# HarmoniaLeo/FRLW-EvD

Hardware: AMD Instinct MI355X
Metric: TAF encode throughput (Mevents/s) (higher is better)
Workload: dtype f32

## Files before the change

frlw-evd_amd/csrc/taf_split.h:

```cpp
#pragma once
#include "taf_column.h"
#include "taf_partition.h"
#include <type_traits>

namespace {
struct TileP {
    int H, W, twl, thl, tiles_x, T, K, n_windows, wb, flip;
    uint32_t win;
    const uint32_t *rec;
    uint32_t *rec2;
    const uint32_t *base;
    uint32_t *sub;
    uint32_t *sub_end;
    const uint32_t *seg0;
    uint32_t *segcnt;
    int pairs;
    int direct;
    int seg_grid;
    uint32_t tile_max;
    const float *tlut;
    const uint32_t *leaky_thr;
    FastHeader *hdr;
    double rcp;
    float *state;
    float *view_f32;
    uint8_t *out_u8;
    uint32_t *wst, *wst_flag;
};

__device__ __forceinline__ int pair_of_segment(const uint32_t *seg0, int pairs, uint32_t seg)
{
    int lo = 0, hi = pairs;
    while (hi - lo > 1) {
        const int mid = (lo + hi) >> 1;
        if (seg0[mid] <= seg) lo = mid; else hi = mid;
    }
    return lo;
}

__device__ __forceinline__ void count_subtiles(const uint32_t *rec, uint32_t beg, uint32_t end, uint32_t (*wtot)[kFW])
{
    const int tid = threadIdx.x, wv = tid >> 6;
    for (uint32_t c0 = beg; c0 < end; c0 += 8 * kFT) {
        uint32_t v[8];
#pragma unroll
        for (int u = 0; u < 8; ++u) {
            const uint32_t i = c0 + (uint32_t)(u * kFT + tid);
            v[u] = rec[i < end ? i : end - 1u];
        }
#pragma unroll
        for (int u = 0; u < 8; ++u)
            if (c0 + (uint32_t)(u * kFT + tid) < end) atomicAdd(&wtot[wv][(v[u] & (kCells - 1)) >> 8], 1u);
    }
}

__device__ __forceinline__ void split_count_segment(const TileP &q, uint32_t seg, uint32_t (*wtot)[kFW])
{
    const int tid = threadIdx.x, wv = tid >> 6;
    if (seg >= q.seg0[q.pairs]) return;
    const int g = pair_of_segment(q.seg0, q.pairs, seg);
    const uint32_t beg = q.base[g] + (seg - q.seg0[g]) * (uint32_t)kSplitSeg;
    const uint32_t end = q.base[g + 1] - beg < (uint32_t)kSplitSeg ? q.base[g + 1] : beg + kSplitSeg;
    if (tid < kFW * kFW) (&wtot[0][0])[tid] = 0u;
    __syncthreads();
    count_subtiles(q.rec, beg, end, wtot);
    __syncthreads();
    if (tid < kFW) {
        uint32_t t = 0;
#pragma unroll
        for (int w = 0; w < kFW; ++w) t += wtot[w][tid];
        q.segcnt[(long long)seg * kFW + tid] = t;
    }
}

constexpr int kWholeChunks = FRLW_WHOLE_SEGS;
constexpr int kWholeBatches = kWholeChunks * kSplitSeg / kWave;
constexpr int kWholeRow = kWholeBatches + 1;

template <bool CM>
__global__ __launch_bounds__(kFT) __attribute__((amdgpu_waves_per_eu(8, 8))) void kf_split_whole(TileP q, CmP cm, SeqTab S)
{
    constexpr int RPT = kSplitSeg / kFT;
    constexpr int kColWords = 2 * kColMax + 1 + kSplitWhole / 32 + 1;
    constexpr int kPoolTail = CM && kColWords > kSplitSeg ? kColWords - kSplitSeg : 0;
    __shared__ __attribute__((aligned(16))) uint32_t pool[kFW * kWholeRow + kSplitSeg + kPoolTail];
    uint32_t *scnt = pool, *stage = pool + kFW * kWholeRow;
    __shared__ uint32_t wtot[kFW][kFW];
    __shared__ uint32_t vtot[kFW];
    __shared__ uint32_t vbeg[kFW][kFW];
    __shared__ uint32_t cE[kFW][kFW], cD[kFW][kFW];
    __shared__ uint32_t s_start, s_first;
    __shared__ int s_unsorted;
    __shared__ int s_fw[kWholeChunks][kFW], s_lw[kWholeChunks][kFW];
    __shared__ uint32_t s_wst[CM ? kFW * (FRLW_MAX_WINDOWS + 1) : 1];
    const int tid = threadIdx.x, lane = tid & 63, wv = tid >> 6;
    const int32_t status0 = q.hdr->status;
    if (!CM && status0 != 0) return;
    const int blk = (int)blockIdx.x;
    if (!CM && blk >= q.pairs) {
        const uint32_t nseg = q.seg0[q.pairs];
        for (uint32_t seg = (uint32_t)(blk - q.pairs); seg < nseg; seg += (uint32_t)q.seg_grid) {
            split_count_segment(q, seg, wtot);
            __syncthreads();
        }
        return;
    }
    const int g = CM ? (int)xcd_owned_index(blockIdx.x, gridDim.x) : blk;
    uint32_t beg, n;
    uint32_t m[kWholeChunks][RPT];
    if (CM) {
        uint32_t *colL = stage, *colD = stage + kColMax + 1;
        uint16_t *idx = (uint16_t *)(stage + 2 * kColMax + 1);
        const int s = g / q.T, C = S.chunk0[s + 1] - S.chunk0[s];
        for (int i = tid; i < kFW * kWholeRow; i += kFT) scnt[i] = 0u;
        n = col_load<kFT>(cm, S, s, g - s * q.T, colL, colD, &wtot[0][0]);
        if (status0 != 0) return;
        if (n == 0u) {
            if (tid < kFW) { q.sub[(long long)g * kFW + tid] = 0u; q.sub_end[(long long)g * kFW + tid] = 0u; }
            if (q.wst && tid == 0) q.wst_flag[g] = 0u;
            return;
        }
        const bool hot = n > q.tile_max;
        if (tid == 0) {
            s_start = atomicAdd(&q.hdr->rec_cursor, n);
            if (hot) s_first = atomicAdd(&q.hdr->seg_cursor, (n + kSplitSeg - 1) / kSplitSeg);
            if (q.wst && hot) q.wst_flag[g] = 0u;
            s_unsorted = 0;
        }
        if (q.wst && !hot) {
            if (tid < kWholeChunks * kFW) { (&s_fw[0][0])[tid] = -1; (&s_lw[0][0])[tid] = -1; }
            for (int i = tid; i < kFW * (q.n_windows + 1); i += kFT) s_wst[i] = 0xffffffffu;
        }
        if (hot) {
            __syncthreads();
            const uint32_t nseg = (n + kSplitSeg - 1) / kSplitSeg, first = s_first;
            if (tid == 0) { cm.hot_start[g] = s_start; cm.hot_seg0[g] = first; }
            for (uint32_t k = tid; k < nseg; k += kFT)
                if (first + k < (uint32_t)cm.max_segs) cm.segdesc[first + k] = (uint32_t)g;
            return;
        }
        col_index<kFT>(colL, C, 0u, n, idx);
        __syncthreads();
        const uint32_t wvs = (uint32_t)__builtin_amdgcn_readfirstlane(wv);
        {
            const __amdgpu_buffer_rsrc_t rsrc = __builtin_amdgcn_make_buffer_rsrc((void *)cm.rec, 0, 0xffffffffu, 0x00020000);
#pragma unroll
            for (int c = 0; c < kWholeChunks; ++c) {
#pragma unroll
                for (int u = 0; u < RPT; ++u) {
                    const uint32_t i = (uint32_t)(c * kSplitSeg + u * kFT + tid), ic = i < n ? i : n - 1u;
                    const uint32_t i0 = (uint32_t)(c * kSplitSeg + u * kFT) + wvs * kWave;
                    uint32_t off = 0u;
                    if (i0 < n) {
                        const uint32_t last = i0 + 63u < n ? i0 + 63u : n - 1u;
                        uint32_t cs = (uint32_t)__builtin_amdgcn_readfirstlane((int)idx[i0 >> 4]);
                        uint32_t lnext = (uint32_t)__builtin_amdgcn_readfirstlane((int)colL[cs + 1]);
                        while (lnext <= i0) { ++cs; lnext = (uint32_t)__builtin_amdgcn_readfirstlane((int)colL[cs + 1]); }
                        if (lnext > last) off = (uint32_t)__builtin_amdgcn_readfirstlane((int)colD[cs]) + ic;
                        else off = col_addr(colL, colD, idx[ic >> 4], ic);
                    }
                    m[c][u] = (uint32_t)__builtin_amdgcn_raw_buffer_load_b32(rsrc, (int)(off << 2), 0, 0);
                }
            }
        }
        beg = (uint32_t)__builtin_amdgcn_readfirstlane((int)s_start);
    } else {
        beg = q.base[g];
        const uint32_t end = q.base[g + 1];
        if (g == q.pairs - 1 && tid == 0) q.sub[(long long)q.pairs * kFW] = end;
        if (end - beg > whole_max_of(q.pairs)) return;
        n = end - beg;
        if (n == 0u) {
            if (tid < kFW) q.sub[(long long)g * kFW + tid] = beg;
            return;
        }
#pragma unroll
        for (int c = 0; c < kWholeChunks; ++c)
#pragma unroll
            for (int u = 0; u < RPT; ++u) {
                const uint32_t i = (uint32_t)(c * kSplitSeg + u * kFT + tid);
                m[c][u] = q.rec[beg + (i < n ? i : n - 1u)];
            }
    }
    if (!CM) {
        for (int i = tid; i < kFW * kWholeRow; i += kFT) scnt[i] = 0u;
        __syncthreads();
    }
    uint32_t rk[kWholeChunks][RPT / 4];
#pragma unroll
    for (int c = 0; c < kWholeChunks; ++c) {
#pragma unroll
        for (int u4 = 0; u4 < RPT / 4; ++u4) rk[c][u4] = 0u;
#pragma unroll
        for (int u = 0; u < RPT; ++u) {
            const uint32_t i0 = (uint32_t)(c * kSplitSeg + u * kFT + wv * kWave);
            if (i0 < n) {
                const bool valid = i0 + (uint32_t)lane < n;
                const uint32_t b = valid ? (m[c][u] & (kCells - 1)) >> 8 : (uint32_t)(lane & 15);
                const uint32_t t = atomicAdd(&scnt[b * kWholeRow + (c * RPT + u) * kFW + wv], valid ? 1u : 0u);
                rk[c][u >> 2] |= t << (8 * (u & 3));
            }
        }
    }
    __syncthreads();
    {
        uint32_t carry = 0;
#pragma unroll
        for (int k = 0; k < kWholeBatches / kWave; ++k) {
            if ((uint32_t)(k * kWave * kWave) < n) {
                const uint32_t v = scnt[wv * kWholeRow + k * kWave + lane];
                const uint32_t inc = wave_incl_scan(v);
                scnt[wv * kWholeRow + k * kWave + lane] = carry + inc - v;
                carry += __shfl(inc, kWave - 1);
            }
        }
        if (lane == 0) vtot[wv] = carry;
    }
    __syncthreads();
    {
        const uint32_t t = vtot[lane & 15];
        uint32_t inc = t;
#pragma unroll
        for (int o2 = 1; o2 < kFW; o2 <<= 1) {
            const uint32_t u = __shfl_up(inc, o2);
            if ((lane & 15) >= o2) inc += u;
        }
        if (lane < kFW) {
            vbeg[wv][lane] = beg + inc - t;
            if (wv == 0) {
                q.sub[(long long)g * kFW + lane] = beg + inc - t;
                if (CM) q.sub_end[(long long)g * kFW + lane] = beg + inc;
            }
        }
        LDS_FENCE();
    }
    const bool wtab = CM && q.wst != nullptr;
#pragma unroll
    for (int c = 0; c < kWholeChunks; ++c) {
        if ((uint32_t)(c * kSplitSeg) >= n) break;
        const uint32_t nch = n - (uint32_t)(c * kSplitSeg) < (uint32_t)kSplitSeg ? n - (uint32_t)(c * kSplitSeg) : (uint32_t)kSplitSeg;
        {
            const int b = lane & 15;
            const uint32_t p0 = scnt[b * kWholeRow + c * (kSplitSeg / kWave)];
            const uint32_t p1 = (uint32_t)((c + 1) * kSplitSeg) < n ? scnt[b * kWholeRow + (c + 1) * (kSplitSeg / kWave)] : vtot[b];
            const uint32_t cnt = p1 - p0;
            uint32_t inc = cnt;
#pragma unroll
            for (int o2 = 1; o2 < kFW; o2 <<= 1) {
                const uint32_t u = __shfl_up(inc, o2);
                if (b >= o2) inc += u;
            }
            if (lane < kFW) {
                cE[wv][lane] = (inc - cnt) - p0;
                cD[wv][lane] = vbeg[wv][lane] + p0 - (inc - cnt);
            }
            LDS_FENCE();
        }
#pragma unroll
        for (int u = 0; u < RPT; ++u) {
            const uint32_t i = (uint32_t)(u * kFT + tid);
            if (i < nch) {
                const uint32_t b = (m[c][u] & (kCells - 1)) >> 8;
                const uint32_t t = (rk[c][u >> 2] >> (8 * (u & 3))) & 255u;
                stage[cE[wv][b] + scnt[b * kWholeRow + (c * RPT + u) * kFW + wv] + t] = m[c][u];
            }
        }
        __syncthreads();
#pragma unroll
        for (int u = 0; u < RPT; ++u) {
            const uint32_t i = (uint32_t)(u * kFT + tid);
            if (i < nch) {
                const uint32_t r = stage[i];
                q.rec2[cD[wv][(r & (kCells - 1)) >> 8] + i] = r;
            }
        }
        if (wtab) {
            const uint32_t dmask = (((1u << q.wb) - 1u) << kCellBits) | (uint32_t)(kCells - 1) >> 8 << 8;
            uint32_t cand = 0u;
#pragma unroll
            for (int u0 = 0; u0 < RPT; u0 += 2) {
                uint32_t r[2], rp[2];
#pragma unroll
                for (int k = 0; k < 2; ++k) {
                    const uint32_t i = (uint32_t)((u0 + k) * kFT + tid);
                    r[k] = stage[i];
                    rp[k] = stage[(i - 1u) & (kSplitSeg - 1)];
                }
#pragma unroll
                for (int k = 0; k < 2; ++k) asm volatile("" : "+v"(r[k]), "+v"(rp[k]));
#pragma unroll
                for (int k = 0; k < 2; ++k) {
                    const uint32_t i = (uint32_t)((u0 + k) * kFT + tid);
                    cand |= (i < nch && (((r[k] ^ rp[k]) & dmask) != 0u || i == 0u || i == nch - 1u) ? 1u : 0u) << (u0 + k);
                }
            }
            while (cand) {
                const int u = __builtin_ctz(cand);
                cand &= cand - 1u;
                const uint32_t i = (uint32_t)(u * kFT + tid);
                const uint32_t r = stage[i], rp = stage[i > 0u ? i - 1u : 0u];
                const int bsub = (int)((r & (kCells - 1)) >> 8), bp = (int)((rp & (kCells - 1)) >> 8);
                const int wc = (int)__builtin_amdgcn_ubfe(r, kCellBits, q.wb), wpn = (int)__builtin_amdgcn_ubfe(rp, kCellBits, q.wb);
                const bool same = i > 0u && bp == bsub;
                if (!same || wc != wpn) atomicMin(&s_wst[bsub * (q.n_windows + 1) + wc], cD[wv][bsub] + i - vbeg[wv][bsub]);
                if (same && wc < wpn) s_unsorted = 1;
                if (!same) { s_fw[c][bsub] = wc; if (i > 0u) s_lw[c][bp] = wpn; }
                if (i == nch - 1u) s_lw[c][bsub] = wc;
            }
        }
        if (wtab && (uint32_t)((c + 1) * kSplitSeg) >= n) LDS_BARRIER();
        else __syncthreads();
    }
    if (wtab) {
        if (tid < kFW) {
            int prev = -1;
            for (int c = 0; c < kWholeChunks; ++c)
                if (s_fw[c][tid] >= 0) { if (s_fw[c][tid] < prev) s_unsorted = 1; prev = s_lw[c][tid]; }
        }
        uint32_t *const wr = q.wst + (long long)g * kFW * (q.n_windows + 1);
        for (int i = tid; i < kFW * (q.n_windows + 1); i += kFT) wr[i] = s_wst[i];
        LDS_BARRIER();
        if (tid == 0) q.wst_flag[g] = s_unsorted ? 2u : 1u;
    }
}

constexpr int kSplitRpt = kSplitSeg / kFT;
struct PlaceLds {
    uint32_t scnt[kSplitRpt][kFW][kFW];
    uint32_t vtot[kFW];
    uint32_t stot[kFW], sdst[kFW];
    uint32_t cE[kFW][kFW], cD[kFW][kFW];
    uint32_t stage[kSplitSeg];
};

struct ColLds {
    uint32_t L[kColMax + 1], D[kColMax];
    uint16_t idx[kSplitSeg / 16];
    uint32_t wsum[kFW + 1];
};

template <bool CM>
__device__ __forceinline__ void split_place_segment(const TileP &q, uint32_t seg, PlaceLds &L, const CmP &cm, const SeqTab &S, ColLds *cl)
{
    constexpr int RPT = kSplitRpt, NE = RPT * kFW;
    const int tid = threadIdx.x, lane = tid & 63, wv = tid >> 6;
    int g;
    uint32_t beg, nrec, seg_first, seg_last, tile_start;
    if (CM) {
        g = __builtin_amdgcn_readfirstlane((int)cm.segdesc[seg]);
        const int s = g / q.T;
        const uint32_t n = col_load<kFT>(cm, S, s, g - s * q.T, cl->L, cl->D, cl->wsum);
        seg_first = (uint32_t)__builtin_amdgcn_readfirstlane((int)cm.hot_seg0[g]);
        seg_last = seg_first + (n + kSplitSeg - 1) / kSplitSeg;
        beg = (seg - seg_first) * (uint32_t)kSplitSeg;
        nrec = n - beg < (uint32_t)kSplitSeg ? n - beg : (uint32_t)kSplitSeg;
        tile_start = (uint32_t)__builtin_amdgcn_readfirstlane((int)cm.hot_start[g]);
        col_index<kFT>(cl->L, S.chunk0[s + 1] - S.chunk0[s], beg, beg + nrec, cl->idx);
    } else {
        g = pair_of_segment(q.seg0, q.pairs, seg);
        beg = q.base[g] + (seg - q.seg0[g]) * (uint32_t)kSplitSeg;
        const uint32_t end = q.base[g + 1] - beg < (uint32_t)kSplitSeg ? q.base[g + 1] : beg + kSplitSeg;
        nrec = end - beg;
        seg_first = q.seg0[g];
        seg_last = q.seg0[g + 1];
        tile_start = q.base[g];
    }
    for (int i = tid; i < RPT * kFW * kFW; i += kFT) (&L.scnt[0][0][0])[i] = 0u;
    uint32_t before = 0, total = 0;
    for (uint32_t sg = seg_first + lane; sg < seg_last; sg += kWave) {
        const uint32_t c = q.segcnt[(long long)sg * kFW + wv];
        total += c;
        if (sg < seg) before += c;
    }
#pragma unroll
    for (int o2 = 32; o2 >= 1; o2 >>= 1) { before += __shfl_xor(before, o2); total += __shfl_xor(total, o2); }
    if (lane == 0) L.vtot[wv] = total;
    __syncthreads();
    uint32_t vstart = tile_start;
    for (int k = 0; k < wv; ++k) vstart += L.vtot[k];
    if (seg == seg_first && lane == 0) {
        q.sub[(long long)g * kFW + wv] = vstart;
        if (CM) q.sub_end[(long long)g * kFW + wv] = vstart + total;
    }
    uint32_t m[RPT], rk[RPT];
    const uint32_t wvs = (uint32_t)__builtin_amdgcn_readfirstlane(wv);
#pragma unroll
    for (int u = 0; u < RPT; ++u) {
        const uint32_t i = (uint32_t)(u * kFT + tid);
        if (CM) {
            const uint32_t ic = i < nrec ? i : nrec - 1u;
            const uint32_t v = cm.rec[col_addr_wave(cl->L, cl->D, cl->idx, beg, (uint32_t)(u * kFT) + wvs * kWave, ic, nrec)];
            m[u] = i < nrec ? v : 0u;
        } else {
            m[u] = i < nrec ? q.rec[beg + i] : 0u;
        }
    }
#pragma unroll
    for (int u = 0; u < RPT; ++u) {
        const uint32_t i = (uint32_t)(u * kFT + tid);
        rk[u] = 0u;
        if (i < nrec) rk[u] = atomicAdd(&L.scnt[u][wv][(m[u] & (kCells - 1)) >> 8], 1u);
    }
    __syncthreads();
    {
        uint32_t v0 = 0, v1 = 0;
        const int e0 = 2 * lane, e1 = 2 * lane + 1;
        if (e0 < NE) v0 = L.scnt[e0 / kFW][e0 % kFW][wv];
        if (e1 < NE) v1 = L.scnt[e1 / kFW][e1 % kFW][wv];
        const uint32_t inc = wave_incl_scan(v0 + v1);
        const uint32_t ex = inc - (v0 + v1);
        if (e0 < NE) L.scnt[e0 / kFW][e0 % kFW][wv] = ex;
        if (e1 < NE) L.scnt[e1 / kFW][e1 % kFW][wv] = ex + v0;
        if (lane == kWave - 1) { L.stot[wv] = inc; L.sdst[wv] = vstart + before; }
    }
    __syncthreads();
    {
        const int b = lane & 15;
        const uint32_t cnt = L.stot[b];
        uint32_t inc = cnt;
#pragma unroll
        for (int o2 = 1; o2 < kFW; o2 <<= 1) {
            const uint32_t u = __shfl_up(inc, o2);
            if (b >= o2) inc += u;
        }
        if (lane < kFW) { L.cE[wv][lane] = inc - cnt; L.cD[wv][lane] = L.sdst[lane] - (inc - cnt); }
        LDS_FENCE();
    }
#pragma unroll
    for (int u = 0; u < RPT; ++u) {
        const uint32_t i = (uint32_t)(u * kFT + tid);
        if (i < nrec) {
            const uint32_t b = (m[u] & (kCells - 1)) >> 8;
            L.stage[L.cE[wv][b] + L.scnt[u][wv][b] + rk[u]] = m[u];
        }
    }
    __syncthreads();
#pragma unroll
    for (int u = 0; u < RPT; ++u) {
        const uint32_t i = (uint32_t)(u * kFT + tid);
        if (i < nrec) {
            const uint32_t r = L.stage[i];
            q.rec2[L.cD[wv][(r & (kCells - 1)) >> 8] + i] = r;
        }
    }
}

template <bool CM>
__global__ __launch_bounds__(kFT) __attribute__((amdgpu_waves_per_eu(8, 8))) void kf_split_place(TileP q, CmP cm, SeqTab S)
{
    __shared__ PlaceLds L;
    __shared__ typename std::conditional<CM, ColLds, uint32_t>::type clmem;
    ColLds *cl = reinterpret_cast<ColLds *>(&clmem);
    if (q.hdr->status != 0) return;
    uint32_t nseg = CM ? q.hdr->seg_cursor : q.seg0[q.pairs];
    if (CM && nseg > (uint32_t)cm.max_segs) nseg = (uint32_t)cm.max_segs;
    for (uint32_t seg = blockIdx.x; seg < nseg; seg += gridDim.x) {
        split_place_segment<CM>(q, seg, L, cm, S, cl);
        __syncthreads();
    }
}

__global__ __launch_bounds__(kFT) __attribute__((amdgpu_waves_per_eu(8, 8))) void kf_segcount_cm(TileP q, CmP cm, SeqTab S)
{
    __shared__ ColLds cl;
    __shared__ uint32_t wtot[kFW][kFW];
    const int tid = threadIdx.x, wv = tid >> 6;
    if (q.hdr->status != 0) return;
    uint32_t nseg = q.hdr->seg_cursor;
    if (nseg > (uint32_t)cm.max_segs) nseg = (uint32_t)cm.max_segs;
    for (uint32_t seg = blockIdx.x; seg < nseg; seg += gridDim.x) {
        const int g = __builtin_amdgcn_readfirstlane((int)cm.segdesc[seg]), s = g / q.T;
        const uint32_t n = col_load<kFT>(cm, S, s, g - s * q.T, cl.L, cl.D, cl.wsum);
        const uint32_t beg = (seg - (uint32_t)__builtin_amdgcn_readfirstlane((int)cm.hot_seg0[g])) * (uint32_t)kSplitSeg;
        const uint32_t nrec = n - beg < (uint32_t)kSplitSeg ? n - beg : (uint32_t)kSplitSeg;
        col_index<kFT>(cl.L, S.chunk0[s + 1] - S.chunk0[s], beg, beg + nrec, cl.idx);
        if (tid < kFW * kFW) (&wtot[0][0])[tid] = 0u;
        __syncthreads();
        uint32_t v[kSplitRpt];
        const uint32_t wvs = (uint32_t)__builtin_amdgcn_readfirstlane(wv);
#pragma unroll
        for (int u = 0; u < kSplitRpt; ++u) {
            const uint32_t i = (uint32_t)(u * kFT + tid), ic = i < nrec ? i : nrec - 1u;
            v[u] = cm.rec[col_addr_wave(cl.L, cl.D, cl.idx, beg, (uint32_t)(u * kFT) + wvs * kWave, ic, nrec)];
        }
#pragma unroll
        for (int u = 0; u < kSplitRpt; ++u)
            if ((uint32_t)(u * kFT + tid) < nrec) atomicAdd(&wtot[wv][(v[u] & (kCells - 1)) >> 8], 1u);
        __syncthreads();
        if (tid < kFW) {
            uint32_t t = 0;
#pragma unroll
            for (int w = 0; w < kFW; ++w) t += wtot[w][tid];
            q.segcnt[(long long)seg * kFW + tid] = t;
        }
        __syncthreads();
    }
}
}
```

frlw-evd_amd/csrc/taf_walk.h:

```cpp
#pragma once
#include "taf_fifo.h"
#include "taf_split.h"

namespace {
__device__ __forceinline__ void fifo_step_half(float (&st)[4], bool upper, bool has, uint32_t n, float mean)
{
    const bool hit = n != 0u;
    const float up = __builtin_bit_cast(float, __builtin_amdgcn_update_dpp(0, __builtin_bit_cast(int, st[0]), 0x101, 0xf, 0xf, false));
#pragma unroll
    for (int k = 0; k < 4; ++k) {
        const float nxt = k < 3 ? st[k + 1] : (upper ? 0.0f : up);
        const float v = (hit ? nxt : st[k]) - 1.0f;
        const float nv = (hit && upper && k == 3) ? mean : v;
        st[k] = has ? nv : st[k];
    }
}

constexpr int kWalkWaves = 8;
constexpr int kWalkThreads = kWalkWaves * kWave;
constexpr int kWalkRpt = 4;
constexpr int kWalkChunk = kWalkRpt * kWave;
constexpr int kWalkSlots = 4;
constexpr int kWalkWaveWords = kWalkSlots * kSubCells + kSubCells / 2;

constexpr int kWalkListCap = 3584;
template <bool K8, bool CMD = false>
__global__ __launch_bounds__(kWalkThreads) __attribute__((amdgpu_waves_per_eu(8, 8))) void kf_taf_walk(TileP q, CmP cm, SeqTab S)
{
    __shared__ __attribute__((aligned(16))) uint32_t s_area[kWalkWaves][kWalkWaveWords];
    __shared__ uint32_t wstart[FRLW_MAX_WINDOWS + 1];
    __shared__ uint32_t thr[kLeakyTableWords];
    __shared__ int s_unsorted;
    __shared__ __attribute__((aligned(16))) uint32_t s_list[CMD ? kWalkListCap : 4];
    const int tid = threadIdx.x, lane = tid & 63, wv = tid >> 6;
    const int sg = CMD ? (int)xcd_owned_index(blockIdx.x, gridDim.x) : (int)blockIdx.x, g = sg / kFW, sub = sg - g * kFW;
    const int s = g / q.T, tile = g - s * q.T;
    const int32_t status0 = q.hdr->status;
    const unsigned long long wmask = q.hdr->wmask[s];
    const uint32_t mul_bad0 = q.hdr->mul_bad;
    uint32_t beg = 0u, end = 0u;
    uint32_t wtab = 0u;
    if (!CMD) {
        beg = q.sub[sg];
        end = q.sub_end ? q.sub_end[sg] : ((sub == kFW - 1 && !q.direct) ? q.base[g + 1] : q.sub[sg + 1]);
        if (q.wst) wtab = q.wst_flag[g];
    }
    if (status0 != 0) return;
    WPROF_INIT();
    const int K = K8 ? 8 : q.K;
    const int NW = q.n_windows;
    const uint32_t *list = q.rec2;
    if (CMD) {
        uint32_t *colL = &s_area[0][0], *colD = colL + (kColDirect + 1);
        static_assert(2 * (kColDirect + 1) <= kWalkWaves * kWalkWaveWords, "the column fits");
        const int C = S.chunk0[s + 1] - S.chunk0[s];
        const uint32_t n = col_load<kWalkThreads>(cm, S, s, sg - s * cm.TB, colL, colD, wstart);
        const bool in_lds = n <= (uint32_t)kWalkListCap;
        uint32_t *dstl;
        if (in_lds) {
            beg = 0u;
            dstl = s_list;
            list = s_list;
        } else {
            if (tid == 0) wstart[0] = atomicAdd(&q.hdr->rec_cursor, n);
            __syncthreads();
            beg = (uint32_t)__builtin_amdgcn_readfirstlane((int)wstart[0]);
            dstl = q.rec2 + beg;
        }
        end = beg + n;
        const int g16 = tid >> 4, l16 = tid & 15;
        for (int c0 = g16; c0 < C; c0 += 4 * (kWalkThreads / 16)) {
            uint32_t v[4], at[4], cnt[4];
#pragma unroll
            for (int u = 0; u < 4; ++u) {
                const int c = c0 + u * (kWalkThreads / 16), cc = c < C ? c : C - 1;
                const uint32_t lo = colL[cc];
                cnt[u] = c < C ? colL[cc + 1] - lo : 0u;
                at[u] = lo;
                v[u] = cm.rec[colD[cc] + lo + ((uint32_t)l16 < cnt[u] ? (uint32_t)l16 : 0u)];
            }
#pragma unroll
            for (int u = 0; u < 4; ++u) {
                if ((uint32_t)l16 < cnt[u]) dstl[at[u] + l16] = v[u];
                if (cnt[u] > 16u) {
                    const int c = c0 + u * (kWalkThreads / 16);
                    const uint32_t d = colD[c];
                    for (uint32_t j = 16u + l16; j < cnt[u]; j += 16u) dstl[at[u] + j] = cm.rec[d + at[u] + j];
                }
            }
        }
        __syncthreads();
    }
    const int ty = tile / q.tiles_x, tx = tile - ty * q.tiles_x;
    const int x0 = tx << q.twl, y0 = ty << q.thl, tw1 = (1 << q.twl) - 1;
    const long long plane = (long long)q.H * q.W;
    const bool owner = tid < kSubCells;
    auto row_of = [&](int t, bool &in_frame) -> float * {
        asm volatile("" : "+v"(t));
        const int c = t & (kSubCells - 1), p2 = sub * (kSubCells / 2) + (c >> 1);
        const int yy = y0 + (p2 >> q.twl), xx = x0 + (p2 & tw1);
        in_frame = t < kSubCells && yy < q.H && xx < q.W;
        return q.state + (((long long)s * plane + (long long)yy * q.W + xx) * 2 + (c & 1)) * K;
    };
    float st[kMaxK];
    float row_touch = 0.0f;
    {
        bool in_frame;
        const float *r = row_of(tid, in_frame);
        if (in_frame) row_touch = r[0];
    }

    uint32_t first_w = 0u;
    unsigned long long nonempty = 0ull;
    bool general;
    const bool use_mul = mul_bad0 == 0u;
    const double rcp = q.rcp;
    const uint32_t wfield = (1u << q.wb) - 1u;
    const int rshift = kCellBits + q.wb;
    {
        uint2 *z = (uint2 *)&s_area[wv][0];
        static_assert(kWalkWaveWords % (2 * kWave) == 0, "whole 8-byte sweeps");
#pragma unroll
        for (int i = 0; i < kWalkWaveWords / 2 / kWave; ++i) z[i * kWave + lane] = make_uint2(0u, 0u);
    }
    if (!CMD && wtab != 0u) {
        const uint32_t *wrow = q.wst + (long long)sg * (NW + 1);
        const uint32_t fw0 = wrow[lane < NW ? lane : NW];
        uint32_t list_touch = 0u;
        for (uint32_t i = beg + 32u * (uint32_t)tid; i < end; i += 32u * kWalkThreads) list_touch |= list[i];
        asm volatile("" ::"v"(list_touch));
        first_w = fw0 != 0xffffffffu ? beg + fw0 : end;
        nonempty = __ballot(lane < NW && fw0 != 0xffffffffu);
        general = wtab == 2u;
        asm volatile("" ::"v"(row_touch));
        WPROF(0);
        WPROF(1);
    } else {
    for (int i = tid; i <= NW; i += kWalkThreads) wstart[i] = end;
    if (tid == 0) s_unsorted = 0;
    __syncthreads();
    WPROF(0);
    {
        const uint32_t n_list = end - beg;
        for (uint32_t c0 = beg & ~3u; c0 < end; c0 += 4 * kWalkThreads) {
            const uint32_t i0 = c0 + 4u * (uint32_t)tid, il = i0 < end ? i0 : (end - 1u) & ~3u;
            const uint4 v4 = *(const uint4 *)(list + il);
            const uint32_t pv = list[il > beg ? il - 1u : beg];
            const uint32_t w0 = __builtin_amdgcn_ubfe(v4.x, kCellBits, q.wb), w1 = __builtin_amdgcn_ubfe(v4.y, kCellBits, q.wb);
            const uint32_t w2 = __builtin_amdgcn_ubfe(v4.z, kCellBits, q.wb), w3 = __builtin_amdgcn_ubfe(v4.w, kCellBits, q.wb);
            const uint32_t wp = il > beg ? __builtin_amdgcn_ubfe(pv, kCellBits, q.wb) : 0xffffffffu;
            const bool full = n_list >= 4u && il - beg <= n_list - 4u;
            if (full) {
                if (w0 != wp || w1 != w0 || w2 != w1 || w3 != w2) {
                    if (w0 != wp) { atomicMin(&wstart[w0], il); if (wp != 0xffffffffu && w0 < wp) s_unsorted = 1; }
                    if (w1 != w0) { atomicMin(&wstart[w1], il + 1u); if (w1 < w0) s_unsorted = 1; }
                    if (w2 != w1) { atomicMin(&wstart[w2], il + 2u); if (w2 < w1) s_unsorted = 1; }
                    if (w3 != w2) { atomicMin(&wstart[w3], il + 3u); if (w3 < w2) s_unsorted = 1; }
                }
            } else {
                const uint32_t ws[5] = {wp, w0, w1, w2, w3};
#pragma unroll
                for (int e = 0; e < 4; ++e) {
                    const uint32_t k = il + (uint32_t)e;
                    if (k - beg < n_list) {
                        const bool first = k == beg;
                        if (first || ws[e + 1] != ws[e]) {
                            atomicMin(&wstart[ws[e + 1]], k);
                            if (!first && ws[e + 1] < ws[e]) s_unsorted = 1;
                        }
                    }
                }
            }
        }
    }
    __syncthreads();
    asm volatile("" ::"v"(row_touch));
    WPROF(1);
    general = s_unsorted != 0;
    first_w = wstart[lane < NW ? lane : NW];
    nonempty = __ballot(lane < NW && first_w != end);
    }
    if (general && tid == 0) atomicAdd(&q.hdr->filtered_tiles, 1u);
    WPROF(2);

    float *rplane = (float *)&s_area[wv][0];
    uint32_t *cnt = &s_area[wv][kWalkSlots * kSubCells];
    const float4 zero4 = make_float4(0.0f, 0.0f, 0.0f, 0.0f);
#pragma nounroll
    for (int g0 = 0; g0 < NW; g0 += kWalkWaves) {
        const int w = g0 + wv;
        float sum[4] = {0.0f, 0.0f, 0.0f, 0.0f};
        uint32_t num[4] = {0u, 0u, 0u, 0u};
        if (g0 > 0) {
            ((float4 *)rplane)[lane] = zero4;
            ((float4 *)rplane)[kWave + lane] = zero4;
        }
        if (w < NW) {
            uint32_t lo = beg, hi = end;
            if (!general) {
                const unsigned long long at = nonempty >> w, behind = w + 1 < 64 ? nonempty >> (w + 1) : 0ull;
                lo = at ? (uint32_t)__builtin_amdgcn_readlane((int)first_w, w + __builtin_ctzll(at)) : end;
                hi = behind ? (uint32_t)__builtin_amdgcn_readlane((int)first_w, w + 1 + __builtin_ctzll(behind)) : end;
            }
#pragma nounroll
            for (uint32_t ptr = lo; ptr < hi; ptr += kWalkChunk) {
                uint32_t m[kWalkRpt], rk[kWalkRpt];
                float val[kWalkRpt];
#pragma unroll
                for (int u = 0; u < kWalkRpt; ++u) {
                    const uint32_t i = ptr + (uint32_t)(u * kWave + lane);
                    m[u] = list[i < hi ? i : hi - 1u];
                }
#pragma unroll
                for (int u = 0; u < kWalkRpt; ++u) {
                    const bool take = ptr + (uint32_t)(u * kWave + lane) < hi && (int)((m[u] >> kCellBits) & wfield) == w;
                    rk[u] = 0xffffffffu;
                    if (take) {
                        const uint32_t lc = m[u] & 255u, sh = (lc & 1u) << 4;
                        rk[u] = (atomicAdd(&cnt[lc >> 1], 1u << sh) >> sh) & 0xffffu;
                    }
                }
                if (use_mul) {
#pragma unroll
                    for (int u = 0; u < kWalkRpt; ++u) val[u] = (float)((double)(m[u] >> rshift) * rcp) - 1.0f;
                } else {
#pragma unroll
                    for (int u = 0; u < kWalkRpt; ++u) {
                        const uint32_t r = m[u] >> rshift;
                        val[u] = q.tlut[r < q.win ? r : q.win];
                    }
                }
                LDS_FENCE();
                const uint2 np = ((const uint2 *)cnt)[lane];
                LDS_FENCE();
                ((uint2 *)cnt)[lane] = make_uint2(0u, 0u);
                const uint4 nn = make_uint4(np.x & 0xffffu, np.x >> 16, np.y & 0xffffu, np.y >> 16);
                const uint32_t n01 = nn.x > nn.y ? nn.x : nn.y, n23 = nn.z > nn.w ? nn.z : nn.w, nmax = n01 > n23 ? n01 : n23;
#pragma nounroll
                for (uint32_t base = 0u;;) {
#pragma unroll
                    for (int u = 0; u < kWalkRpt; ++u) {
                        const uint32_t rr = rk[u] - base;
                        if (rr < (uint32_t)kWalkSlots) rplane[rr * kSubCells + (m[u] & 255u)] = val[u];
                    }
                    LDS_FENCE();
#pragma unroll
                    for (int r = 0; r < kWalkSlots; ++r) {
                        const float4 pr = ((const float4 *)(rplane + r * kSubCells))[lane];
                        LDS_FENCE();
                        ((float4 *)(rplane + r * kSubCells))[lane] = zero4;
                        sum[0] = sum[0] + pr.x;
                        sum[1] = sum[1] + pr.y;
                        sum[2] = sum[2] + pr.z;
                        sum[3] = sum[3] + pr.w;
                    }
                    base += (uint32_t)kWalkSlots;
                    if (__ballot(nmax > base) == 0ull) break;
                }
                num[0] += nn.x; num[1] += nn.y; num[2] += nn.z; num[3] += nn.w;
                LDS_FENCE();
            }
        }
        ((float4 *)rplane)[lane] = make_float4(fifo_mean(num[0], sum[0]), fifo_mean(num[1], sum[1]), fifo_mean(num[2], sum[2]), fifo_mean(num[3], sum[3]));
        ((uint4 *)(rplane + kSubCells))[lane] = make_uint4(num[0], num[1], num[2], num[3]);
        static_assert(kLeakyTableWords <= kWalkThreads, "one word per thread");
        uint32_t thr_v = 0u;
        if (g0 == 0 && tid < kLeakyTableWords) thr_v = q.leaky_thr[tid];
        if (g0 == 0) {
#pragma unroll
            for (int kk = 0; kk < kMaxK; ++kk) st[kk] = 0.0f;
            bool ok;
            const float *srow = row_of(tid, ok);
            if (ok) {
                if (K8) {
                    const float4 a = ((const float4 *)srow)[0], b = ((const float4 *)srow)[1];
                    st[0] = a.x; st[1] = a.y; st[2] = a.z; st[3] = a.w; st[4] = b.x; st[5] = b.y; st[6] = b.z; st[7] = b.w;
                } else {
#pragma unroll
                    for (int kk = 0; kk < kMaxK; ++kk)
                        if (kk < K) st[kk] = srow[kk];
                }
            }
        }
        WPROF(3);
        __syncthreads();
        WPROF(4);
        if (owner) {
            uint32_t rn[kWalkWaves];
            float rm[kWalkWaves];
#pragma unroll
            for (int ws = 0; ws < kWalkWaves; ++ws) {
                rn[ws] = s_area[ws][kSubCells + tid];
                rm[ws] = __uint_as_float(s_area[ws][tid]);
            }
#pragma unroll
            for (int ws = 0; ws < kWalkWaves; ++ws)
                if (g0 + ws < NW && ((wmask >> (g0 + ws)) & 1ull)) fifo_step(st, K, true, rn[ws], rm[ws]);
        }
        if (g0 == 0 && tid < kLeakyTableWords) thr[tid] = thr_v;
        __syncthreads();
        WPROF(5);
    }

    uint8_t *ob = (uint8_t *)&s_area[0][0];
    float4 *rowst = (float4 *)&s_area[1][0];
    static_assert(kWalkWaveWords * 4 >= 2 * kMaxK * (kSubCells / 2) && (kWalkWaves - 1) * kWalkWaveWords * 4 >= kSubCells * 32, "staging fits");
    if (K8 && owner) {
        rowst[2 * tid] = make_float4(st[0], st[1], st[2], st[3]);
        rowst[2 * tid + 1] = make_float4(st[4], st[5], st[6], st[7]);
    }
    const int pol = tid & 1;
    {
        bool ok;
        float *srow = row_of(tid, ok);
        if (ok) {
            if (!K8) {
#pragma unroll
                for (int k = 0; k < kMaxK; ++k)
                    if (k < K) srow[k] = st[k];
            }
            if (q.view_f32) {
                float *vw = q.view_f32 + (long long)s * 2 * K * plane + ((srow - q.state) / (2 * K) - (long long)s * plane);
#pragma unroll
                for (int k = 0; k < kMaxK; ++k)
                    if (k < K) vw[(long long)(2 * k + pol) * plane] = st[k];
            }
        }
    }
    if (q.out_u8) {
        if (owner) {
            uint8_t lv[kMaxK];
            leaky_u8_bucket_n<kMaxK>(st, thr, lv);
#pragma unroll
            for (int k = 0; k < kMaxK; ++k) {
                if (k < K) {
                    const int ko = q.flip ? (K - 1 - k) : k;
                    ob[(2 * ko + pol) * (kSubCells / 2) + (tid >> 1)] = lv[k];
                }
            }
        }
    }
    WPROF(6);
    if (K8 || q.out_u8) __syncthreads();
    WPROF(7);
    if (K8) {
        const int c2 = tid >> 1, pt2 = sub * (kSubCells / 2) + (c2 >> 1);
        const int py2 = y0 + (pt2 >> q.twl), px2 = x0 + (pt2 & tw1);
        if (py2 < q.H && px2 < q.W)
            ((float4 *)(q.state + (((long long)s * plane + (long long)py2 * q.W + px2) * 2 + (c2 & 1)) * 8))[tid & 1] = rowst[tid];
    }
    if (q.out_u8) {
        for (int c = tid; c < 2 * K * 8; c += kWalkThreads) {
            const int pl = c >> 3, part = c & 7;
            const int p16 = sub * (kSubCells / 2) + 16 * part;
            const int y = y0 + (p16 >> q.twl), x = x0 + (p16 & tw1);
            if (y >= q.H || x >= q.W) continue;
            const uint8_t *src = ob + pl * (kSubCells / 2) + 16 * part;
            uint8_t *dst = q.out_u8 + ((long long)s * 2 * K + pl) * plane + (long long)y * q.W + x;
            if (x + 16 <= q.W && (((uintptr_t)dst) & 15u) == 0) {
                *(uint4 *)dst = *(const uint4 *)src;
            } else {
                const int nv = q.W - x < 16 ? q.W - x : 16;
                for (int e = 0; e < nv; ++e) dst[e] = src[e];
            }
        }
    }
    WPROF(8);
    WPROF_END();
}
}
```

Measured before the change: 74340.

## Use per-16-record block table for column address lookup in split kernel

Replaces the per-record column search (idx table plus a wave-uniform while loop over column boundaries) with a precomputed per-16-record BtEntry table. Each entry encodes a base address and at most one column boundary inside the block, and falls back to walking the column list when a block spans more boundaries. Chunks beyond n are also skipped early. In the walk kernel, the window-start row is loaded earlier and the list prefetch-touch loop is removed. This adds table-building work and LDS use, and blocks that need the fallback walk are slower than the fast path.

```diff
diff --git a/frlw-evd_amd/csrc/taf_blocktab.h b/frlw-evd_amd/csrc/taf_blocktab.h
--- /dev/null
+++ b/frlw-evd_amd/csrc/taf_blocktab.h
@@ -0,0 +1,45 @@
+#pragma once
+#include <stdint.h>
+
+#if defined(__HIPCC__)
+#define FRLW_BT_HD __host__ __device__ __forceinline__
+#else
+#define FRLW_BT_HD inline
+#endif
+
+namespace frlw_bt {
+constexpr uint32_t kBtFallback = 0xffffffffu;
+constexpr int kBtCols = 1024;
+
+struct alignas(8) BtEntry {
+    uint32_t a, w;
+};
+
+FRLW_BT_HD void bt_build_run(const uint32_t *L, const uint32_t *D, int C, int c, uint32_t n, BtEntry *tab)
+{
+    const uint32_t hi = L[c + 1];
+    uint32_t i = (L[c] + 15u) & ~15u;
+    if (i >= hi) return;
+    const uint32_t da = D[c];
+    for (; hi - i >= 16u; i += 16u) tab[i >> 4] = BtEntry{da, 0u};
+    if (i >= hi) return;
+    BtEntry e{da, 0u};
+    if (hi < n) {
+        int b = c + 1;
+        while (b < C - 1 && L[b + 1] == hi) ++b;
+        const uint32_t end = n - i < 16u ? n : i + 16u, delta = D[b] - da;
+        const uint32_t w = delta << 4 | (hi - i);
+        if (L[b + 1] < end || delta >= (1u << 28) || w == kBtFallback) e = BtEntry{(uint32_t)c, kBtFallback};
+        else e.w = w;
+    }
+    tab[i >> 4] = e;
+}
+
+FRLW_BT_HD uint32_t bt_addr(BtEntry e, uint32_t i) { return e.a + i + ((i & 15u) >= (e.w & 15u) ? e.w >> 4 : 0u); }
+
+FRLW_BT_HD uint32_t bt_walk(const uint32_t *L, const uint32_t *D, uint32_t c, uint32_t i)
+{
+    while (L[c + 1] <= i) ++c;
+    return D[c] + i;
+}
+}
diff --git a/frlw-evd_amd/csrc/taf_split.h b/frlw-evd_amd/csrc/taf_split.h
--- a/frlw-evd_amd/csrc/taf_split.h
+++ b/frlw-evd_amd/csrc/taf_split.h
@@ -1,4 +1,5 @@
 #pragma once
+#include "taf_blocktab.h"
 #include "taf_column.h"
 #include "taf_partition.h"
 #include <type_traits>
@@ -81,6 +82,7 @@
 __global__ __launch_bounds__(kFT) __attribute__((amdgpu_waves_per_eu(8, 8))) void kf_split_whole(TileP q, CmP cm, SeqTab S)
 {
     constexpr int RPT = kSplitSeg / kFT;
+    constexpr int kBtGroup = 4;
     constexpr int kColWords = 2 * kColMax + 1 + kSplitWhole / 32 + 1;
     constexpr int kPoolTail = CM && kColWords > kSplitSeg ? kColWords - kSplitSeg : 0;
     __shared__ __attribute__((aligned(16))) uint32_t pool[kFW * kWholeRow + kSplitSeg + kPoolTail];
@@ -109,9 +111,12 @@
     uint32_t beg, n;
     uint32_t m[kWholeChunks][RPT];
     if (CM) {
-        uint32_t *colL = stage, *colD = stage + kColMax + 1;
+        const int s = g / q.T, C = S.chunk0[s + 1] - S.chunk0[s];
+        const bool tabled = C <= frlw_bt::kBtCols && S.ev0[S.n_seq] - S.ev0[0] < (1ll << 28);
+        static_assert(2 * frlw_bt::kBtCols + 2 + kSplitWhole / 16 * 2 <= kSplitSeg, "column + table inside the staging area");
+        uint32_t *colL = stage, *colD = stage + (tabled ? frlw_bt::kBtCols : kColMax) + 1;
         uint16_t *idx = (uint16_t *)(stage + 2 * kColMax + 1);
-        const int s = g / q.T, C = S.chunk0[s + 1] - S.chunk0[s];
+        frlw_bt::BtEntry *tab = (frlw_bt::BtEntry *)(stage + 2 * frlw_bt::kBtCols + 2);
         for (int i = tid; i < kFW * kWholeRow; i += kFT) scnt[i] = 0u;
         n = col_load<kFT>(cm, S, s, g - s * q.T, colL, colD, &wtot[0][0]);
         if (status0 != 0) return;
@@ -139,13 +144,48 @@
                 if (first + k < (uint32_t)cm.max_segs) cm.segdesc[first + k] = (uint32_t)g;
             return;
         }
-        col_index<kFT>(colL, C, 0u, n, idx);
+        if (tabled) {
+            for (int c = tid; c < C; c += kFT) frlw_bt::bt_build_run(colL, colD, C, c, n, tab);
+        } else {
+            col_index<kFT>(colL, C, 0u, n, idx);
+        }
         __syncthreads();
         const uint32_t wvs = (uint32_t)__builtin_amdgcn_readfirstlane(wv);
         {
             const __amdgpu_buffer_rsrc_t rsrc = __builtin_amdgcn_make_buffer_rsrc((void *)cm.rec, 0, 0xffffffffu, 0x00020000);
+            if (tabled) {
+#pragma unroll
+                for (int c = 0; c < kWholeChunks; ++c) {
+                    if ((uint32_t)(c * kSplitSeg) >= n) break;
+#pragma unroll
+                    for (int u0 = 0; u0 < RPT; u0 += kBtGroup) {
+                        frlw_bt::BtEntry e[kBtGroup];
+                        uint32_t ic[kBtGroup], wmax = 0u;
+#pragma unroll
+                        for (int k = 0; k < kBtGroup; ++k) {
+                            const uint32_t i = (uint32_t)(c * kSplitSeg + (u0 + k) * kFT + tid);
+                            ic[k] = i < n ? i : n - 1u;
+                            e[k] = tab[ic[k] >> 4];
+                        }
+#pragma unroll
+                        for (int k = 0; k < kBtGroup; ++k) wmax = e[k].w > wmax ? e[k].w : wmax;
+                        if (__builtin_expect(__ballot(wmax == frlw_bt::kBtFallback) == 0ull, 1)) {
+#pragma unroll
+                            for (int k = 0; k < kBtGroup; ++k)
+                                m[c][u0 + k] = (uint32_t)__builtin_amdgcn_raw_buffer_load_b32(rsrc, (int)(frlw_bt::bt_addr(e[k], ic[k]) << 2), 0, 0);
+                        } else {
+#pragma unroll
+                            for (int k = 0; k < kBtGroup; ++k) {
+                                const uint32_t off = e[k].w == frlw_bt::kBtFallback ? frlw_bt::bt_walk(colL, colD, e[k].a, ic[k]) : frlw_bt::bt_addr(e[k], ic[k]);
+                                m[c][u0 + k] = (uint32_t)__builtin_amdgcn_raw_buffer_load_b32(rsrc, (int)(off << 2), 0, 0);
+                            }
+                        }
+                    }
+                }
+            } else {
 #pragma unroll
             for (int c = 0; c < kWholeChunks; ++c) {
+                if ((uint32_t)(c * kSplitSeg) >= n) break;
 #pragma unroll
                 for (int u = 0; u < RPT; ++u) {
                     const uint32_t i = (uint32_t)(c * kSplitSeg + u * kFT + tid), ic = i < n ? i : n - 1u;
@@ -161,6 +201,7 @@
                     }
                     m[c][u] = (uint32_t)__builtin_amdgcn_raw_buffer_load_b32(rsrc, (int)(off << 2), 0, 0);
                 }
+            }
             }
         }
         beg = (uint32_t)__builtin_amdgcn_readfirstlane((int)s_start);
diff --git a/frlw-evd_amd/csrc/taf_walk.h b/frlw-evd_amd/csrc/taf_walk.h
--- a/frlw-evd_amd/csrc/taf_walk.h
+++ b/frlw-evd_amd/csrc/taf_walk.h
@@ -40,10 +40,14 @@
     const uint32_t mul_bad0 = q.hdr->mul_bad;
     uint32_t beg = 0u, end = 0u;
     uint32_t wtab = 0u;
+    uint32_t fw_row = 0xffffffffu;
     if (!CMD) {
         beg = q.sub[sg];
         end = q.sub_end ? q.sub_end[sg] : ((sub == kFW - 1 && !q.direct) ? q.base[g + 1] : q.sub[sg + 1]);
-        if (q.wst) wtab = q.wst_flag[g];
+        if (q.wst) {
+            wtab = q.wst_flag[g];
+            fw_row = q.wst[(long long)sg * (q.n_windows + 1) + (lane < q.n_windows ? lane : q.n_windows)];
+        }
     }
     if (status0 != 0) return;
     WPROF_INIT();
@@ -124,11 +128,7 @@
         for (int i = 0; i < kWalkWaveWords / 2 / kWave; ++i) z[i * kWave + lane] = make_uint2(0u, 0u);
     }
     if (!CMD && wtab != 0u) {
-        const uint32_t *wrow = q.wst + (long long)sg * (NW + 1);
-        const uint32_t fw0 = wrow[lane < NW ? lane : NW];
-        uint32_t list_touch = 0u;
-        for (uint32_t i = beg + 32u * (uint32_t)tid; i < end; i += 32u * kWalkThreads) list_touch |= list[i];
-        asm volatile("" ::"v"(list_touch));
+        const uint32_t fw0 = fw_row;
         first_w = fw0 != 0xffffffffu ? beg + fw0 : end;
         nonempty = __ballot(lane < NW && fw0 != 0xffffffffu);
         general = wtab == 2u;
```

Result: faster. 78520, median of 6 (+5.6%).
